# eriklindernoren/PyTorch-GAN

Measured on NVIDIA H100. Metric: DCGAN 64x64 images/sec (full G+D step), higher is better.
Workload: dtype tf32 (fp32 storage, fp32 accumulate)

## Files before the change

pytorch-gan_b200/csrc/narrow_block.cu:

```cuda
#include "tc_common.cuh"
#include <string.h>

namespace b200gan {

struct NbBn {
  const double *stats;
  const float *gamma, *beta;
  float eps;
  double count;
  int groups;
};

__device__ __forceinline__ void nb_bn_consts(const NbBn &bn, int C, int c, float &mean, float &rstd, float &sc,
                                             float &sh, double *var_out = nullptr, int grp = 0) {
  const double *st = bn.stats + (size_t)grp * 2 * C;
  const double m = st[c] / bn.count;
  double var = st[C + c] / bn.count - m * m;
  if (var < 0.0) var = 0.0;
  if (var_out) *var_out = var;
  rstd = (float)(1.0 / sqrt(var + (double)bn.eps));
  mean = (float)m;
  const float ga = bn.gamma ? bn.gamma[c] : 1.f, be = bn.beta ? bn.beta[c] : 0.f;
  sc = ga * rstd;
  sh = be - mean * sc;
// ... 6 lines not shown
    double var;
    nb_bn_consts(bn, C, c, mean, rstd, sc, sh, &var, grp);
    const double unbiased = bn.count > 1.0 ? var * bn.count / (bn.count - 1.0) : var;
    m_run = (1.f - momentum) * m_run + momentum * mean;
    v_run = (1.f - momentum) * v_run + momentum * (float)unbiased;
  }
  rm[c] = m_run;
  rv[c] = v_run;
}

__device__ __forceinline__ float nb_act(float v, int act, float slope) {
  if (act == B200GAN_ACT_LRELU) return v > 0.f ? v : v * slope;
  if (act == B200GAN_ACT_RELU) return fmaxf(v, 0.f);
  if (act == B200GAN_ACT_TANH) return tanhf(v);
  if (act == B200GAN_ACT_SIGMOID) return 1.f / (1.f + expf(-v));
  return v;
}
__device__ __forceinline__ float nb_act_grad(float a, int act, float slope) {
  if (act == B200GAN_ACT_LRELU) return a > 0.f ? 1.f : slope;
  if (act == B200GAN_ACT_RELU) return a > 0.f ? 1.f : 0.f;
  return 1.f;
}

__device__ __forceinline__ int ceil_div_dev(int a, int b) { return (a + b - 1) / b; }
__device__ __forceinline__ float warp_sum(float v) {
#pragma unroll
  for (int o = 16; o > 0; o >>= 1) v += __shfl_xor_sync(0xffffffffu, v, o);
  return v;
}

constexpr int NB_MAXC = 128;
constexpr int NB_MAX_GROUPS = 4;

__device__ __forceinline__ void nb_stage(float *dst, int CP, const float *src_img, int h0, int w0, int rows, int cols, int C,
                                         int H, int W, const float *sc_s, const float *sh_s, bool reflect, int tid) {
  if ((C & 3) == 0) {
    const int C4 = C >> 2, total = rows * cols * C4;
    for (int i = tid; i < total; i += 256) {
      const int c4 = i % C4, pix = i / C4;
      const int pc = pix % cols, pr = pix / cols;
      int ih = h0 + pr, iw = w0 + pc;
      if (reflect) {
        ih = reflect_idx(ih, H);
        iw = reflect_idx(iw, W);
      }
      float4 v = make_float4(0.f, 0.f, 0.f, 0.f);
      if (src_img && ih >= 0 && ih < H && iw >= 0 && iw < W) {
        v = __ldg(reinterpret_cast<const float4 *>(src_img + ((int64_t)ih * W + iw) * C) + c4);
        if (sc_s) {
          const float4 a = *reinterpret_cast<const float4 *>(sc_s + 4 * c4), b = *reinterpret_cast<const float4 *>(sh_s + 4 * c4);
          v.x = fmaf(v.x, a.x, b.x); v.y = fmaf(v.y, a.y, b.y); v.z = fmaf(v.z, a.z, b.z); v.w = fmaf(v.w, a.w, b.w);
        }
      }
      *reinterpret_cast<float4 *>(dst + (int64_t)pix * CP + 4 * c4) = v;
    }
  } else {
    const int total = rows * cols * C;
    for (int i = tid; i < total; i += 256) {
      const int cc = i % C, pix = i / C;
      const int pc = pix % cols, pr = pix / cols;
      int ih = h0 + pr, iw = w0 + pc;
      if (reflect) {
        ih = reflect_idx(ih, H);
        iw = reflect_idx(iw, W);
      }
      float v = 0.f;
      if (src_img && ih >= 0 && ih < H && iw >= 0 && iw < W) {
        v = __ldg(src_img + ((int64_t)ih * W + iw) * C + cc);
        if (sc_s) v = fmaf(v, sc_s[cc], sh_s[cc]);
      }
      dst[(int64_t)pix * CP + cc] = v;
    }
  }
}

struct NbTile {
  int TN, TR, TQ, TP, KG, KB;
  int tiles_r, tiles_q;
};

struct NbFprop2 {
  const float *x, *wp, *bias, *cs;
  float *y;
  double *out_stats;
  NbBn in_bn;
  float *rm, *rv;
  long long *nbt;
  float momentum;
  int N, H, W, C, P, Q, K, R, S, stride, pad_t, pad_l;
  float slope;
  int act;
  NbTile t;
  int PR, PC, CP;
  int reflect;
  int rtf;
  int groups;
};
template <int KT, int PT>
__global__ void __launch_bounds__(256)
nbk_fprop2_kernel(const __grid_constant__ NbFprop2 p) {
  extern __shared__ __align__(16) float nsm[];
  const NbTile &t = p.t;
  const int taps = p.R * p.S;
  float *w_s = nsm;
  float *x_s = w_s + (size_t)taps * p.C * t.KB;
  float *sc_s = x_s + (((size_t)t.TN * p.PR * p.PC * p.CP + 3) & ~(size_t)3);
  float *sh_s = sc_s + ((p.C + 3) & ~3);
  float *red = sh_s + ((p.C + 3) & ~3);
  const int tid = threadIdx.x, lane = tid & 31, warp = tid >> 5;
  const bool has_in = p.in_bn.stats != nullptr;
  const int grp = (int)((blockIdx.x / (t.tiles_q * t.tiles_r)) * t.TN) / (p.N / p.groups);
  for (int cc = tid; cc < p.C; cc += 256) {
    float mean, rstd, sc = 1.f, sh = 0.f;
    if (has_in) {
      nb_bn_consts(p.in_bn, p.C, cc, mean, rstd, sc, sh, nullptr, grp);
      if (blockIdx.x == 0 && blockIdx.y == 0 && p.rm) nb_update_running(p.in_bn, p.C, cc, p.rm, p.rv, p.momentum);
    }
    sc_s[cc] = sc;
    sh_s[cc] = sh;
  }
  if (has_in && blockIdx.x == 0 && blockIdx.y == 0 && tid == 0 && p.nbt) *p.nbt += p.in_bn.groups;
  const int kbase = blockIdx.y * t.KB;
  {
    const int KB4 = t.KB >> 2, total = taps * p.C * KB4;
#pragma unroll 4
    for (int i = tid; i < total; i += 256) {
      const int col = i % KB4, row = i / KB4;
      reinterpret_cast<float4 *>(w_s)[i] = __ldg(reinterpret_cast<const float4 *>(p.wp + (int64_t)row * p.K + kbase) + col);
    }
  }
  __syncthreads();
  int tile = blockIdx.x;
  const int tq = tile % t.tiles_q;
  tile /= t.tiles_q;
  const int tr = tile % t.tiles_r;
  const int n0 = (tile / t.tiles_r) * t.TN;
  const int p0 = tr * t.TR, q0 = tq * t.TQ;
  for (int li = 0; li < t.TN; ++li) {
    const int n = n0 + li;
    nb_stage(x_s + (size_t)li * p.PR * p.PC * p.CP, p.CP, n < p.N ? p.x + (int64_t)n * p.H * p.W * p.C : nullptr,
             p0 * p.stride - p.pad_t, q0 * p.stride - p.pad_l, p.PR, p.PC, p.C, p.H, p.W, has_in ? sc_s : nullptr, sh_s,
             p.reflect != 0, tid);
  }
  __syncthreads();

  const int TPX = t.TP / PT;
  const int lpx = tid % TPX, kgi = tid / TPX;
  int xoff[PT];
  int64_t yoff[PT];
  int nn[PT];
#pragma unroll
  for (int i = 0; i < PT; ++i) {
    const int lp = lpx + i * TPX;
    const int lq = lp % t.TQ, lr = (lp / t.TQ) % t.TR, li = lp / (t.TQ * t.TR);
    const int n = n0 + li, po = p0 + lr, qo = q0 + lq;
    xoff[i] = ((li * p.PR + lr * p.stride) * p.PC + lq * p.stride) * p.CP;
    nn[i] = n;
    yoff[i] = (n < p.N && po < p.P && qo < p.Q) ? ((int64_t)(n * p.P + po) * p.Q + qo) * p.K : -1;
  }
  float acc[PT][KT];
#pragma unroll
  for (int i = 0; i < PT; ++i)
#pragma unroll
    for (int j = 0; j < KT; ++j) acc[i][j] = 0.f;
  const float *wb = w_s + kgi * KT;
  const int KB = t.KB;
  for (int r = 0; r < p.R; ++r) {
    for (int s = 0; s < p.S; ++s) {
      const float *xt = x_s + (r * p.PC + s) * p.CP;
      const float *wt = wb + (size_t)(r * p.S + s) * p.C * KB;
      if ((p.C & 3) == 0) {
#pragma unroll 2
        for (int c = 0; c < p.C; c += 4) {
          float xs[PT][4];
#pragma unroll
          for (int i = 0; i < PT; ++i) {
            const float4 xv = *reinterpret_cast<const float4 *>(xt + xoff[i] + c);
// ... 6 lines not shown
            for (int u = 0; u < KT / 4; ++u) {
              const float4 w4 = *reinterpret_cast<const float4 *>(wr + 4 * u);
#pragma unroll
              for (int i = 0; i < PT; ++i) {
                acc[i][4 * u + 0] = fmaf(xs[i][j], w4.x, acc[i][4 * u + 0]);
                acc[i][4 * u + 1] = fmaf(xs[i][j], w4.y, acc[i][4 * u + 1]);
                acc[i][4 * u + 2] = fmaf(xs[i][j], w4.z, acc[i][4 * u + 2]);
                acc[i][4 * u + 3] = fmaf(xs[i][j], w4.w, acc[i][4 * u + 3]);
              }
            }
          }
        }
      } else {
        for (int c = 0; c < p.C; ++c) {
          float xs[PT];
#pragma unroll
          for (int i = 0; i < PT; ++i) xs[i] = xt[xoff[i] + c];
          const float *wr = wt + (size_t)c * KB;
#pragma unroll
          for (int u = 0; u < KT / 4; ++u) {
            const float4 w4 = *reinterpret_cast<const float4 *>(wr + 4 * u);
#pragma unroll
            for (int i = 0; i < PT; ++i) {
              acc[i][4 * u + 0] = fmaf(xs[i], w4.x, acc[i][4 * u + 0]);
              acc[i][4 * u + 1] = fmaf(xs[i], w4.y, acc[i][4 * u + 1]);
              acc[i][4 * u + 2] = fmaf(xs[i], w4.z, acc[i][4 * u + 2]);
              acc[i][4 * u + 3] = fmaf(xs[i], w4.w, acc[i][4 * u + 3]);
            }
          }
        }
      }
    }
  }
  const int k0 = kbase + kgi * KT;
  float s1[KT], s2[KT];
#pragma unroll
  for (int j = 0; j < KT; ++j) s1[j] = s2[j] = 0.f;
#pragma unroll
  for (int i = 0; i < PT; ++i) {
    const bool valid = yoff[i] >= 0;
#pragma unroll
    for (int j = 0; j < KT; ++j) {
      float v = acc[i][j];
      if (p.bias) v += __ldg(p.bias + k0 + j);
      v = nb_act(v, p.act, p.slope);
      if (p.cs && valid) v *= __ldg(p.cs + (int64_t)nn[i] * p.K + k0 + j);
      if (p.rtf) v = round_tf32(v);
      v = valid ? v : 0.f;
      acc[i][j] = v;
      s1[j] += v;
      s2[j] = fmaf(v, v, s2[j]);
    }
    if (valid) {
      float *yo = p.y + yoff[i] + k0;
#pragma unroll
      for (int u = 0; u < KT / 4; ++u)
        *reinterpret_cast<float4 *>(yo + 4 * u) =
            make_float4(acc[i][4 * u], acc[i][4 * u + 1], acc[i][4 * u + 2], acc[i][4 * u + 3]);
    }
  }
  if (p.out_stats) {
#pragma unroll
    for (int j = 0; j < KT; ++j) {
      const float a1 = warp_sum(s1[j]), a2 = warp_sum(s2[j]);
      if (lane == 0) {
        red[warp * 2 * KT + j] = a1;
        red[warp * 2 * KT + KT + j] = a2;
      }
    }
    __syncthreads();
    if (tid < t.KG * 2 * KT) {
      const int g = tid / (2 * KT), idx = tid % (2 * KT), wpg = TPX >> 5;
      float tsum = 0.f;
      for (int wi = 0; wi < wpg; ++wi) tsum += red[(g * wpg + wi) * 2 * KT + idx];
      atomicAdd(p.out_stats + (size_t)grp * 2 * p.K + (idx < KT ? 0 : p.K) + kbase + g * KT + (idx % KT), (double)tsum);
    }
  }
}

struct NbDz {
  const float *g, *a, *cs;
  float *dz, *db;
  NbBn out_bn;
  const double *sums;
  int64_t rows;
  int64_t PQ;
  int K;
  float slope;
  int act;
};
__global__ void __launch_bounds__(256)
nbk_dz_kernel(const __grid_constant__ NbDz p) {
  __shared__ float red[256][4];
  const int tid = threadIdx.x;
  const int K4 = p.K >> 2;
  const int kq = tid % K4;
  const int rows_per_block = 256 / K4;
  const bool has_bn = p.out_bn.stats != nullptr;
  const int grp = blockIdx.y;
  const int64_t grows = p.rows / gridDim.y, grow0 = grp * grows;
  float mean[4], rstd[4], sc[4], m1[4], m2[4];
#pragma unroll
  for (int j = 0; j < 4; ++j) {
    mean[j] = 0.f; rstd[j] = 0.f; sc[j] = 1.f; m1[j] = 0.f; m2[j] = 0.f;
    if (has_bn) {
      float sh;
      nb_bn_consts(p.out_bn, p.K, kq * 4 + j, mean[j], rstd[j], sc[j], sh, nullptr, grp);
      m1[j] = (float)(p.sums[(size_t)grp * 2 * p.K + kq * 4 + j] / p.out_bn.count);
      m2[j] = (float)(p.sums[(size_t)grp * 2 * p.K + p.K + kq * 4 + j] / p.out_bn.count);
    }
// ... 19 lines not shown
      o[j] = dA * csv[j] * nb_act_grad(A[j], p.act, p.slope);
      dbs[j] += o[j];
    }
    *reinterpret_cast<float4 *>(p.dz + off) = make_float4(o[0], o[1], o[2], o[3]);
  }
  if (p.db) {
#pragma unroll
    for (int j = 0; j < 4; ++j) red[tid][j] = dbs[j];
    __syncthreads();
    if (tid < K4) {
      float t4[4] = {0.f, 0.f, 0.f, 0.f};
      for (int r = 0; r < rows_per_block; ++r)
#pragma unroll
        for (int j = 0; j < 4; ++j) t4[j] += red[r * K4 + tid][j];
#pragma unroll
      for (int j = 0; j < 4; ++j) atomicAdd(p.db + tid * 4 + j, t4[j]);
    }
  }
}

struct NbWgrad {
  const float *x, *dz;
  float *dw;
  float *ws;
  int dw_elems;
  NbBn in_bn;
  int N, H, W, C, P, Q, K, R, S, stride, pad_t, pad_l;
  int TN, TR, TQ, tiles_r, tiles_q;
  int PR, PC;
  int SPB, PS;
  int nsets;
  int row_mode;
  int reflect;
};
template <int TAPS>
__global__ void __launch_bounds__(256, 2)
nbk_wgrad_kernel(const __grid_constant__ NbWgrad p) {
  extern __shared__ __align__(16) float nsm[];
  const int tile_px = p.TN * p.TR * p.TQ;
  const int K4 = (p.K + 3) >> 2, KP = K4 * 4;
  const int patch_img = p.PR * p.PC * p.C;
  int *sbase_s = reinterpret_cast<int *>(nsm);
  int *sk_s = sbase_s + p.SPB;
  int *poff_s = sk_s + p.SPB;
  float *x_s = nsm + ((2 * p.SPB + tile_px + 3) & ~3);
  float *dz_s = x_s + (((size_t)p.TN * patch_img + 3) & ~(size_t)3);
  const int Cr = (p.C + 3) & ~3;
  const int groups = p.in_bn.groups, img_per_group = p.N / groups;
  float *sc_s = dz_s + (size_t)tile_px * KP;
  float *sh_s = sc_s + (size_t)groups * Cr;
  const int tid = threadIdx.x;
  const bool has_in = p.in_bn.stats != nullptr;
  for (int i = tid; i < groups * p.C; i += 256) {
    const int gq = i / p.C, cc = i - gq * p.C;
    float mean, rstd, sc = 1.f, sh = 0.f;
    if (has_in) nb_bn_consts(p.in_bn, p.C, cc, mean, rstd, sc, sh, nullptr, gq);
    sc_s[gq * Cr + cc] = sc;
    sh_s[gq * Cr + cc] = sh;
  }
  for (int pix = tid; pix < tile_px; pix += 256) {
    const int lq = pix % p.TQ, lr = (pix / p.TQ) % p.TR, li = pix / (p.TQ * p.TR);
    poff_s[pix] = li * patch_img + ((lr * p.stride) * p.PC + lq * p.stride) * p.C;
  }
  const int RS = p.R * p.S;
  for (int sl = tid; sl < p.SPB; sl += 256) {
    const int set_o = blockIdx.y * p.SPB + sl;
    int base = -1, k0 = 0;
    if (set_o < p.nsets) {
      const int co = set_o % p.C, kgo = (set_o / p.C) % K4;
      const int ro = p.row_mode ? set_o / (p.C * K4) : 0;
      k0 = kgo * 4;
      base = (k0 * p.C + co) * RS + ro * p.S;
    }
    sbase_s[sl] = base;
    sk_s[sl] = k0;
  }
  const int set_local = tid & (p.SPB - 1), psplit = tid / p.SPB;
  const int set = blockIdx.y * p.SPB + set_local;
  const bool set_ok = set < p.nsets;
  const int c = set_ok ? set % p.C : 0, kg = set_ok ? (set / p.C) % K4 : 0;
  const int r_own = (set_ok && p.row_mode) ? set / (p.C * K4) : 0;
  float acc[TAPS][4];
#pragma unroll
  for (int t = 0; t < TAPS; ++t)
#pragma unroll
    for (int j = 0; j < 4; ++j) acc[t][j] = 0.f;
  const int ntiles = ceil_div_dev(p.N, p.TN) * p.tiles_r * p.tiles_q;
  int toff[TAPS];
#pragma unroll
  for (int t = 0; t < TAPS; ++t) toff[t] = p.row_mode ? (r_own * p.PC + t) * p.C : ((t / p.S) * p.PC + (t % p.S)) * p.C;
  __syncthreads();
  for (int tile = blockIdx.x; tile < ntiles; tile += gridDim.x) {
    const int tq = tile % p.tiles_q;
    const int tr = (tile / p.tiles_q) % p.tiles_r;
    const int n0 = (tile / (p.tiles_q * p.tiles_r)) * p.TN;
    const int p0 = tr * p.TR, q0 = tq * p.TQ;
    const int h0 = p0 * p.stride - p.pad_t, w0 = q0 * p.stride - p.pad_l;
    for (int li = 0; li < p.TN; ++li) {
      const int n = n0 + li;
      const int gq = n < p.N ? n / img_per_group : 0;
      nb_stage(x_s + (size_t)li * patch_img, p.C, n < p.N ? p.x + (int64_t)n * p.H * p.W * p.C : nullptr, h0, w0, p.PR, p.PC,
               p.C, p.H, p.W, has_in ? sc_s + gq * Cr : nullptr, sh_s + gq * Cr, p.reflect != 0, tid);
    }
    const int img_px = p.TR * p.TQ;
    if ((p.K & 3) == 0) {
      for (int i = tid; i < tile_px * K4; i += 256) {
        const int k4 = i % K4, pix = i / K4;
        const int li = pix / img_px, rem = pix - li * img_px;
        const int lr = rem / p.TQ, lq = rem - lr * p.TQ;
        float4 v = make_float4(0.f, 0.f, 0.f, 0.f);
        if (n0 + li < p.N && p0 + lr < p.P && q0 + lq < p.Q)
          v = __ldg(reinterpret_cast<const float4 *>(p.dz + ((int64_t)((n0 + li) * p.P + p0 + lr) * p.Q + q0 + lq) * p.K) + k4);
        reinterpret_cast<float4 *>(dz_s)[i] = v;
      }
    } else {
      for (int i = tid; i < tile_px * KP; i += 256) {
        const int k = i % KP, pix = i / KP;
        const int li = pix / img_px, rem = pix - li * img_px;
        const int lr = rem / p.TQ, lq = rem - lr * p.TQ;
        float v = 0.f;
        if (k < p.K && n0 + li < p.N && p0 + lr < p.P && q0 + lq < p.Q)
          v = __ldg(p.dz + ((int64_t)((n0 + li) * p.P + p0 + lr) * p.Q + q0 + lq) * p.K + k);
        dz_s[i] = v;
      }
    }
    __syncthreads();
    if (set_ok) {
      const float *xc = x_s + c;
      const float *dk = dz_s + kg * 4;
#pragma unroll 2
      for (int pix = psplit; pix < tile_px; pix += p.PS) {
        const float4 d4 = *reinterpret_cast<const float4 *>(dk + pix * KP);
        const float *xb = xc + poff_s[pix];
#pragma unroll
        for (int t = 0; t < TAPS; ++t) {
          const float xv = xb[toff[t]];
          acc[t][0] = fmaf(xv, d4.x, acc[t][0]);
          acc[t][1] = fmaf(xv, d4.y, acc[t][1]);
          acc[t][2] = fmaf(xv, d4.z, acc[t][2]);
          acc[t][3] = fmaf(xv, d4.w, acc[t][3]);
        }
      }
    }
    __syncthreads();
  }
  constexpr int TPAD = TAPS | 1;
  float *red = x_s;
#pragma unroll
  for (int j = 0; j < 4; ++j)
#pragma unroll
    for (int t = 0; t < TAPS; ++t) red[((size_t)(psplit * 4 + j) * p.SPB + set_local) * TPAD + t] = acc[t][j];
  __syncthreads();
  const int nout = 4 * p.SPB * TAPS;
  const int kstride = p.C * RS;
  float *slab = p.ws ? p.ws + (size_t)blockIdx.x * p.dw_elems : nullptr;
  for (int o = tid; o < nout; o += 256) {
    const int t = o % TAPS, rest = o / TAPS;
    const int sl = rest & (p.SPB - 1), j = rest / p.SPB;
    const int base = sbase_s[sl];
    if (base < 0) continue;
    if (sk_s[sl] + j >= p.K) continue;
    float sum = 0.f;
    for (int ps = 0; ps < p.PS; ++ps) sum += red[((size_t)(ps * 4 + j) * p.SPB + sl) * TPAD + t];
    const int idx = base + j * kstride + t;
    if (slab) slab[idx] = sum;
    else atomicAdd(p.dw + idx, sum);
  }
}

__global__ void __launch_bounds__(256)
nbk_wgrad_reduce_kernel(const float *__restrict__ ws, float *__restrict__ dw, int elems, int nslabs) {
  __shared__ float part[8][32];
  const int e = blockIdx.x * 32 + (threadIdx.x & 31), ph = threadIdx.x >> 5;
  float a = 0.f;
  if (e < elems) {
#pragma unroll 4
    for (int sl = ph; sl < nslabs; sl += 8) a += __ldg(ws + (size_t)sl * elems + e);
  }
  part[ph][threadIdx.x & 31] = a;
  __syncthreads();
  if (ph == 0 && e < elems) {
    float t = 0.f;
#pragma unroll
    for (int i = 0; i < 8; ++i) t += part[i][threadIdx.x];
    dw[e] = t;
  }
}

struct NbDgrad2 {
  const float *dz, *wp, *a_prev;
  float *g_out;
  double *sums;
  NbBn in_bn;
  int N, H, W, C, P, Q, K, R, S, stride, pad_t, pad_l;
  NbTile t;
  int KP;
  int PRm, PCm;
  int tapsm;
};
template <int KT, int PT>
__global__ void __launch_bounds__(256)
nbk_dgrad2_kernel(const __grid_constant__ NbDgrad2 p) {
  extern __shared__ __align__(16) float nsm[];
  const NbTile &t = p.t;
  float *w_s = nsm;
  float *d_s = w_s + (((size_t)p.tapsm * p.K * t.KB + 3) & ~(size_t)3);
  float *mean_s = d_s + (((size_t)t.TN * p.PRm * p.PCm * p.KP + 3) & ~(size_t)3);
  float *rstd_s = mean_s + ((p.C + 3) & ~3);
  float *red = rstd_s + ((p.C + 3) & ~3);
  const int tid = threadIdx.x, lane = tid & 31, warp = tid >> 5;
  const bool has_in = p.sums != nullptr;
  const int grp = (int)((blockIdx.x / (t.tiles_q * t.tiles_r)) * t.TN) / (p.N / p.in_bn.groups);
  if (has_in) {
    for (int cc = tid; cc < p.C; cc += 256) {
      float sc, sh;
      nb_bn_consts(p.in_bn, p.C, cc, mean_s[cc], rstd_s[cc], sc, sh, nullptr, grp);
    }
  }
  const int st = p.stride;
  const int cls = blockIdx.z;
  const int pa = cls / st, pb = cls % st;
  const int r0 = (pa + p.pad_t) % st, s0 = (pb + p.pad_l) % st;
  const int Rc = r0 < p.R ? (p.R - r0 + st - 1) / st : 0, Sc = s0 < p.S ? (p.S - s0 + st - 1) / st : 0;
  const int Hc = pa < p.H ? (p.H - pa + st - 1) / st : 0, Wc = pb < p.W ? (p.W - pb + st - 1) / st : 0;
  const int oh = (pa + p.pad_t - r0) / st, ow = (pb + p.pad_l - s0) / st;
  const int cbase = blockIdx.y * t.KB;
  const int KB = t.KB;
  if ((KB & 3) == 0) {
    const int KB4 = KB >> 2, total = Rc * Sc * p.K * KB4;
#pragma unroll 4
    for (int i = tid; i < total; i += 256) {
      const int col = i % KB4, row = i / KB4;
      const int k = row % p.K, ti = row / p.K;
      const int r = r0 + st * (ti / Sc), s_ = s0 + st * (ti % Sc);
      reinterpret_cast<float4 *>(w_s)[i] =
          __ldg(reinterpret_cast<const float4 *>(p.wp + ((int64_t)(r * p.S + s_) * p.K + k) * p.C + cbase) + col);
    }
  } else {
    const int total = Rc * Sc * p.K * KB;
    for (int i = tid; i < total; i += 256) {
      const int col = i % KB, row = i / KB;
      const int k = row % p.K, ti = row / p.K;
      const int r = r0 + st * (ti / Sc), s_ = s0 + st * (ti % Sc);
      w_s[i] = __ldg(p.wp + ((int64_t)(r * p.S + s_) * p.K + k) * p.C + cbase + col);
    }
  }
  int tile = blockIdx.x;
  const int tq = tile % t.tiles_q;
  tile /= t.tiles_q;
  const int tr = tile % t.tiles_r;
  const int n0 = (tile / t.tiles_r) * t.TN;
  const int i0 = tr * t.TR, j0 = tq * t.TQ;
  const int PRc = t.TR + (Rc > 0 ? Rc - 1 : 0), PCc = t.TQ + (Sc > 0 ? Sc - 1 : 0);
  for (int li = 0; li < t.TN; ++li) {
    const int n = n0 + li;
    nb_stage(d_s + (size_t)li * PRc * PCc * p.KP, p.KP, n < p.N ? p.dz + (int64_t)n * p.P * p.Q * p.K : nullptr,
             i0 + oh - (Rc - 1), j0 + ow - (Sc - 1), PRc, PCc, p.K, p.P, p.Q, nullptr, nullptr, false, tid);
  }
  __syncthreads();

  const int TPX = t.TP / PT;
  const int lpx = tid % TPX, cgi = tid / TPX;
  int doff[PT];
  int64_t opix[PT];
#pragma unroll
  for (int i = 0; i < PT; ++i) {
    const int lp = lpx + i * TPX;
    const int lq = lp % t.TQ, lr = (lp / t.TQ) % t.TR, li = lp / (t.TQ * t.TR);
    const int n = n0 + li, ci = i0 + lr, cj = j0 + lq;
    doff[i] = ((li * PRc + lr) * PCc + lq) * p.KP;
    opix[i] = (n < p.N && ci < Hc && cj < Wc) ? (int64_t)(n * p.H + pa + st * ci) * p.W + pb + st * cj : -1;
  }
  float acc[PT][KT];
#pragma unroll
  for (int i = 0; i < PT; ++i)
#pragma unroll
    for (int j = 0; j < KT; ++j) acc[i][j] = 0.f;
  const float *wb = w_s + cgi * KT;
  for (int ir = 0; ir < Rc; ++ir) {
    for (int is = 0; is < Sc; ++is) {
      const float *dt = d_s + ((Rc - 1 - ir) * PCc + (Sc - 1 - is)) * p.KP;
      const float *wt = wb + (size_t)(ir * Sc + is) * p.K * KB;
#pragma unroll 2
      for (int k = 0; k < p.K; k += 4) {
        float ds[PT][4];
#pragma unroll
        for (int i = 0; i < PT; ++i) {
          const float4 dv = *reinterpret_cast<const float4 *>(dt + doff[i] + k);
          ds[i][0] = dv.x; ds[i][1] = dv.y; ds[i][2] = dv.z; ds[i][3] = dv.w;
        }
#pragma unroll
        for (int j = 0; j < 4; ++j) {
          const float *wr = wt + (size_t)(k + j) * KB;
          if (KT % 4 == 0) {
#pragma unroll
            for (int u = 0; u < KT / 4; ++u) {
              const float4 w4 = *reinterpret_cast<const float4 *>(wr + 4 * u);
#pragma unroll
              for (int i = 0; i < PT; ++i) {
                acc[i][4 * u + 0] = fmaf(ds[i][j], w4.x, acc[i][4 * u + 0]);
                acc[i][4 * u + 1] = fmaf(ds[i][j], w4.y, acc[i][4 * u + 1]);
                acc[i][4 * u + 2] = fmaf(ds[i][j], w4.z, acc[i][4 * u + 2]);
                acc[i][4 * u + 3] = fmaf(ds[i][j], w4.w, acc[i][4 * u + 3]);
              }
            }
          } else {
#pragma unroll
            for (int u = 0; u < KT; ++u) {
              const float wv = wr[u];
#pragma unroll
              for (int i = 0; i < PT; ++i) acc[i][u] = fmaf(ds[i][j], wv, acc[i][u]);
            }
          }
        }
      }
    }
  }
  const int c0 = cbase + cgi * KT;
  float s1[KT], s2[KT];
#pragma unroll
  for (int j = 0; j < KT; ++j) s1[j] = s2[j] = 0.f;
#pragma unroll
  for (int i = 0; i < PT; ++i) {
    if (opix[i] < 0) continue;
    float *go = p.g_out + opix[i] * p.C + c0;
    if (KT % 4 == 0) {
#pragma unroll
      for (int u = 0; u < KT / 4; ++u)
        *reinterpret_cast<float4 *>(go + 4 * u) =
            make_float4(acc[i][4 * u], acc[i][4 * u + 1], acc[i][4 * u + 2], acc[i][4 * u + 3]);
    } else {
#pragma unroll
      for (int j = 0; j < KT; ++j) go[j] = acc[i][j];
    }
    if (has_in) {
      float ah[KT];
      if (KT % 4 == 0) {
#pragma unroll
        for (int u = 0; u < KT / 4; ++u) {
          const float4 a4 = __ldg(reinterpret_cast<const float4 *>(p.a_prev + opix[i] * p.C + c0) + u);
          ah[4 * u] = a4.x; ah[4 * u + 1] = a4.y; ah[4 * u + 2] = a4.z; ah[4 * u + 3] = a4.w;
        }
      } else {
#pragma unroll
        for (int j = 0; j < KT; ++j) ah[j] = __ldg(p.a_prev + opix[i] * p.C + c0 + j);
      }
#pragma unroll
      for (int j = 0; j < KT; ++j) {
        s1[j] += acc[i][j];
        s2[j] = fmaf(acc[i][j], (ah[j] - mean_s[c0 + j]) * rstd_s[c0 + j], s2[j]);
      }
    }
  }
  if (has_in) {
#pragma unroll
    for (int j = 0; j < KT; ++j) {
      const float a1 = warp_sum(s1[j]), a2 = warp_sum(s2[j]);
      if (lane == 0) {
        red[warp * 2 * KT + j] = a1;
        red[warp * 2 * KT + KT + j] = a2;
      }
    }
    __syncthreads();
    if (tid < t.KG * 2 * KT) {
      const int g = tid / (2 * KT), idx = tid % (2 * KT), wpg = TPX >> 5;
      float tsum = 0.f;
      for (int wi = 0; wi < wpg; ++wi) tsum += red[(g * wpg + wi) * 2 * KT + idx];
      atomicAdd(p.sums + (size_t)grp * 2 * p.C + (idx < KT ? 0 : p.C) + cbase + g * KT + (idx % KT), (double)tsum);
    }
  }
}

struct NbTail {
  const float *a;
  const float *dout;
  float *out;
  float *g;
  double *sums;
  NbBn bn;
  float *rm, *rv;
  long long *nbt;
  float momentum;
  int N, HW, C, nchw;
};
__global__ void __launch_bounds__(256)
nbk_tail_fwd_kernel(const __grid_constant__ NbTail p) {
  __shared__ float sc_s[NB_MAXC], sh_s[NB_MAXC];
  const int tid = threadIdx.x;
  const int grp = blockIdx.y;
  if (tid < p.C) {
    float mean, rstd;
    nb_bn_consts(p.bn, p.C, tid, mean, rstd, sc_s[tid], sh_s[tid], nullptr, grp);
    if (blockIdx.x == 0 && grp == 0 && p.rm) nb_update_running(p.bn, p.C, tid, p.rm, p.rv, p.momentum);
  }
  if (blockIdx.x == 0 && grp == 0 && tid == 0 && p.nbt) *p.nbt += p.bn.groups;
  __syncthreads();
  const int64_t gtotal = (int64_t)(p.N / gridDim.y) * p.HW * p.C, total = (grp + 1) * gtotal;
  for (int64_t i = grp * gtotal + (int64_t)blockIdx.x * 256 + tid; i < total; i += (int64_t)gridDim.x * 256) {
    int c;
    int64_t src;
    if (p.nchw) {
      const int hw = (int)(i % p.HW);
      c = (int)((i / p.HW) % p.C);
// ... 173 lines not shown
  X(3, 2) X(3, 4) X(1, 1)
#define NB_IS_INSTANCE(KT_, PT_) if (pl.KT == KT_ && pl.PT == PT_) return true;
static bool nb_fprop_instance(const NbPlan &pl) {
  NB_FPROP_INSTANCES(NB_IS_INSTANCE)
  return false;
}
static bool nb_dgrad_instance(const NbPlan &pl) {
  NB_DGRAD_INSTANCES(NB_IS_INSTANCE)
  return false;
}
#undef NB_IS_INSTANCE

static int nb_fprop2_launch(const b200gan_conv_geom *g, const NbBn &in_bn, float *rm, float *rv, long long *nbt,
                            float momentum, const float *x, const float *packed, const float *bias, int act, float slope,
                            const float *chan_scale, float *y, double *out_stats, int reflect, int rtf, int groups,
                            cudaStream_t st) {
  B2_CHECK_ARG(groups >= 1 && groups <= NB_MAX_GROUPS && g->N % groups == 0, "nb_fprop: bad statistics group count");
  const NbPlan pl = nb_plan_fprop(g, groups);
  B2_CHECK_ARG(pl.ok, "nb_fprop: no tile plan fits in shared memory");
  B2_CHECK_ARG(nb_fprop_instance(pl), "nb_fprop: no kernel instance for KT=%d PT=%d", pl.KT, pl.PT);
  if (out_stats) B2_CUDA(cudaMemsetAsync(out_stats, 0, (size_t)groups * 2 * g->K * sizeof(double), st));
  NbFprop2 q;
  q.x = x; q.wp = packed; q.bias = bias; q.cs = chan_scale; q.y = y; q.out_stats = out_stats;
  q.in_bn = in_bn; q.rm = rm; q.rv = rv; q.nbt = nbt; q.momentum = momentum;
  q.N = g->N; q.H = g->H; q.W = g->W; q.C = g->C; q.P = g->P; q.Q = g->Q; q.K = g->K; q.R = g->R; q.S = g->S;
  q.stride = g->stride; q.pad_t = g->pad_t; q.pad_l = g->pad_l; q.slope = slope; q.act = act;
  q.t = pl.t;
  q.PR = (pl.t.TR - 1) * g->stride + g->R;
  q.PC = (pl.t.TQ - 1) * g->stride + g->S;
  q.CP = (g->C % 4 == 0) ? g->C + 4 : g->C;
  q.reflect = reflect;
  q.rtf = rtf;
  q.groups = groups;
  dim3 grid((unsigned)(ceil_div(g->N, pl.t.TN) * pl.t.tiles_r * pl.t.tiles_q), (unsigned)(g->K / pl.t.KB));
#define NB_FPROP_CASE(KT_, PT_)                                                                              \
  if (pl.KT == KT_ && pl.PT == PT_) {                                                                        \
    static std::atomic<uint64_t> done{0};                                                                    \
    if (int e = ensure_dynamic_smem(nbk_fprop2_kernel<KT_, PT_>, (int)NB_SMEM_MAX, done)) return e;          \
    nbk_fprop2_kernel<KT_, PT_><<<grid, 256, pl.smem, st>>>(q);                                              \
  }
  NB_FPROP_INSTANCES(NB_FPROP_CASE)
#undef NB_FPROP_CASE
  B2_LAUNCH_CHECK();
  return B200GAN_OK;
}

bool nb_plain_fprop_ok(const b200gan_conv_geom *g) {
  if (!g || g->transposed || g->up != 1) return false;
  if (g->pad_mode != B200GAN_PAD_ZERO && g->pad_mode != B200GAN_PAD_REFLECT) return false;
  if (g->stride != 1 && g->stride != 2) return false;
  if (g->C < 1 || g->C > 8 || g->K < 16 || g->K > NB_MAXC || g->K % 16 != 0) return false;
  if (g->R != g->S || (g->R != 3 && g->R != 4 && g->R != 7)) return false;
  return nb_plan_fprop(g).ok;
}
int nb_plain_fprop(const b200gan_conv_geom *g, const b200gan_epilogue *ep, const float *x, const float *packed, float *y,
                   cudaStream_t st) {
  if ((int64_t)g->N * g->P * g->Q == 0) return B200GAN_OK;
  NbBn none = to_bn(nullptr);
  return nb_fprop2_launch(g, none, nullptr, nullptr, nullptr, 0.f, x, packed, ep ? ep->bias : nullptr,
                          ep ? ep->act : B200GAN_ACT_NONE, ep ? ep->slope : 0.f, ep ? ep->chan_scale : nullptr, y, nullptr,
                          g->pad_mode == B200GAN_PAD_REFLECT ? 1 : 0, ep ? ep->round_tf32 : 0, 1, st);
}
}

extern "C" int b200gan_nb_fprop(const b200gan_conv_geom *g, const b200gan_nb_bn *in_bn, float *running_mean,
                                float *running_var, int64_t *num_batches_tracked, float momentum, const float *x,
// ... 118 lines not shown
  B2_CHECK_ARG(validate_geom(g) == B200GAN_OK && nb_wgrad_ok(g), "nb_wgrad: unsupported geometry");
  B2_CHECK_ARG(x && dz && dw, "nb_wgrad: null pointer");
  return nb_wgrad_run(g, in_bn, x, dz, dw, workspace, as_stream(stream));
}

int b200gan::nb_wgrad_run(const b200gan_conv_geom *g, const b200gan_nb_bn *in_bn, const float *x, const float *dz,
                          float *dw, float *workspace, cudaStream_t st) {
  const int dw_elems = g->K * g->C * g->R * g->S;
  if ((int64_t)g->N * g->P * g->Q == 0) {
    B2_CUDA(cudaMemsetAsync(dw, 0, (size_t)dw_elems * sizeof(float), st));
    return B200GAN_OK;
  }
  const int groups = (in_bn && in_bn->stats && in_bn->groups > 1) ? in_bn->groups : 1;
  B2_CHECK_ARG(g->N % groups == 0, "nb_wgrad: the batch must split evenly into the statistics groups");
  B2_CHECK_ARG(groups == 1 || (groups <= NB_MAX_GROUPS && g->C <= NB_MAXC), "nb_wgrad: too many statistics groups");
  const NbWgPlan w = nb_wgrad_plan(g);
  B2_CHECK_ARG(w.smem <= 96 * 1024, "nb_wgrad: tile does not fit in shared memory");
  const bool use_ws = w.use_ws && workspace != nullptr;
  if (!use_ws) B2_CUDA(cudaMemsetAsync(dw, 0, (size_t)dw_elems * sizeof(float), st));
  NbWgrad p;
  p.x = x; p.dz = dz; p.dw = dw; p.ws = use_ws ? workspace : nullptr; p.dw_elems = dw_elems; p.in_bn = to_bn(in_bn);
  p.N = g->N; p.H = g->H; p.W = g->W; p.C = g->C; p.P = g->P; p.Q = g->Q; p.K = g->K; p.R = g->R; p.S = g->S;
  p.stride = g->stride; p.pad_t = g->pad_t; p.pad_l = g->pad_l;
  p.TN = w.TN; p.TR = w.TR; p.TQ = w.TQ;
  p.tiles_r = ceil_div(g->P, p.TR);
  p.tiles_q = ceil_div(g->Q, p.TQ);
  p.PR = (p.TR - 1) * g->stride + g->R;
  p.PC = (p.TQ - 1) * g->stride + g->S;
  p.row_mode = w.row_mode;
  p.reflect = g->pad_mode == B200GAN_PAD_REFLECT ? 1 : 0;
  p.nsets = w.nsets;
  p.SPB = w.SPB;
  p.PS = w.PS;
  const int taps = g->R * g->S;
  static std::atomic<uint64_t> done9{0}, done16{0}, done7{0};
  dim3 grid((unsigned)w.gx, (unsigned)w.nchunks);
  if (p.row_mode) {
    if (int e = ensure_dynamic_smem(nbk_wgrad_kernel<7>, 96 * 1024, done7)) return e;
    nbk_wgrad_kernel<7><<<grid, 256, w.smem, st>>>(p);
  } else if (taps == 9) {
    if (int e = ensure_dynamic_smem(nbk_wgrad_kernel<9>, 96 * 1024, done9)) return e;
    nbk_wgrad_kernel<9><<<grid, 256, w.smem, st>>>(p);
  } else {
    if (int e = ensure_dynamic_smem(nbk_wgrad_kernel<16>, 96 * 1024, done16)) return e;
    nbk_wgrad_kernel<16><<<grid, 256, w.smem, st>>>(p);
  }
  B2_LAUNCH_CHECK();
  if (use_ws) return nb_wgrad_reduce(workspace, dw, dw_elems, w.gx, st);
  return B200GAN_OK;
}

int b200gan::nb_wgrad_reduce(const float *ws, float *dw, int elems, int nslabs, cudaStream_t st) {
  nbk_wgrad_reduce_kernel<<<(unsigned)ceil_div(elems, 32), 256, 0, st>>>(ws, dw, elems, nslabs);
  B2_LAUNCH_CHECK();
  return B200GAN_OK;
}

namespace b200gan {
static int nb_dgrad2_launch(const b200gan_conv_geom *g, const float *dz, const float *packed, const NbBn &in_bn,
                            const float *a_prev, float *g_out, double *sums, cudaStream_t st) {
  const int st_ = g->stride;
  const int groups = in_bn.stats ? in_bn.groups : 1;
  B2_CHECK_ARG(groups <= NB_MAX_GROUPS && g->N % groups == 0, "nb_dgrad: bad statistics group count");
  const NbPlan pl = nb_plan_dgrad(g, groups);
  B2_CHECK_ARG(pl.ok, "nb_dgrad: no tile plan fits in shared memory");
  B2_CHECK_ARG(nb_dgrad_instance(pl), "nb_dgrad: no kernel instance for KT=%d PT=%d", pl.KT, pl.PT);
  if (sums) B2_CUDA(cudaMemsetAsync(sums, 0, (size_t)groups * 2 * g->C * sizeof(double), st));
  NbDgrad2 q;
  q.dz = dz; q.wp = packed; q.a_prev = a_prev; q.g_out = g_out; q.sums = sums; q.in_bn = in_bn;
  q.N = g->N; q.H = g->H; q.W = g->W; q.C = g->C; q.P = g->P; q.Q = g->Q; q.K = g->K; q.R = g->R; q.S = g->S;
  q.stride = g->stride; q.pad_t = g->pad_t; q.pad_l = g->pad_l;
  q.t = pl.t;
  q.KP = g->K + 4;
  const int Rm = ceil_div(g->R, st_), Sm = ceil_div(g->S, st_);
  q.PRm = pl.t.TR + Rm - 1;
  q.PCm = pl.t.TQ + Sm - 1;
  q.tapsm = Rm * Sm;
  dim3 grid((unsigned)(ceil_div(g->N, pl.t.TN) * pl.t.tiles_r * pl.t.tiles_q), (unsigned)(g->C / pl.t.KB),
            (unsigned)(st_ * st_));
#define NB_DGRAD_CASE(KT_, PT_)                                                                              \
  if (pl.KT == KT_ && pl.PT == PT_) {                                                                        \
    static std::atomic<uint64_t> done{0};                                                                    \
    if (int e = ensure_dynamic_smem(nbk_dgrad2_kernel<KT_, PT_>, (int)NB_SMEM_MAX, done)) return e;          \
    nbk_dgrad2_kernel<KT_, PT_><<<grid, 256, pl.smem, st>>>(q);                                              \
  }
  NB_DGRAD_INSTANCES(NB_DGRAD_CASE)
#undef NB_DGRAD_CASE
  B2_LAUNCH_CHECK();
  return B200GAN_OK;
}

bool nb_plain_dgrad_ok(const b200gan_conv_geom *g) {
  if (!g || g->transposed || g->up != 1 || g->pad_mode != B200GAN_PAD_ZERO) return false;
  if (g->stride != 1 && g->stride != 2) return false;
  if (g->pad_t != g->pad_b || g->pad_l != g->pad_r) return false;
  if (g->C < 1 || g->C > 8 || (g->C != 1 && g->C != 3 && g->C != 6 && g->C % 4 != 0)) return false;
  if (g->K < 4 || g->K > NB_MAXC || g->K % 4 != 0) return false;
  if (g->R * g->S != 9 && g->R * g->S != 16 && !(g->R == 7 && g->S == 7 && g->stride == 1)) return false;
  return nb_plan_dgrad(g).ok;
}
int nb_plain_dgrad(const b200gan_conv_geom *g, const float *dy, const float *packed, float *dx, cudaStream_t st) {
  if ((int64_t)g->N * g->H * g->W == 0) return B200GAN_OK;
  NbBn none = to_bn(nullptr);
  return nb_dgrad2_launch(g, dy, packed, none, nullptr, dx, nullptr, st);
}
}

extern "C" int b200gan_nb_dgrad(const b200gan_conv_geom *g, const float *dz, const float *packed,
                                const b200gan_nb_bn *in_bn, const float *a_prev, float *g_out, double *sums,
                                void *stream) {
// ... 55 lines not shown
```

Baseline: 47140.

## Stage conv tiles with cp.async and overlap loads with BN constant setup

Replaces register-staged global→shared copies of weights, input patches and dz in the narrow-block fprop, wgrad and dgrad kernels with cp.async transfers, issuing them before the per-channel BN constant computation so the two overlap. Input normalization is split into a second in-shared-memory pass after the copy completes, which costs an extra shared read/write and sync when BN is applied. It also adds compile-time-gated clock tracing hooks and an incremental index helper to avoid per-element divisions.

```diff
diff --git a/pytorch-gan_b200/csrc/narrow_block.cu b/pytorch-gan_b200/csrc/narrow_block.cu
--- a/pytorch-gan_b200/csrc/narrow_block.cu
+++ b/pytorch-gan_b200/csrc/narrow_block.cu
@@ -62,44 +62,93 @@
 constexpr int NB_MAXC = 128;
 constexpr int NB_MAX_GROUPS = 4;
 
-__device__ __forceinline__ void nb_stage(float *dst, int CP, const float *src_img, int h0, int w0, int rows, int cols, int C,
-                                         int H, int W, const float *sc_s, const float *sh_s, bool reflect, int tid) {
-  if ((C & 3) == 0) {
-    const int C4 = C >> 2, total = rows * cols * C4;
-    for (int i = tid; i < total; i += 256) {
-      const int c4 = i % C4, pix = i / C4;
-      const int pc = pix % cols, pr = pix / cols;
-      int ih = h0 + pr, iw = w0 + pc;
-      if (reflect) {
-        ih = reflect_idx(ih, H);
-        iw = reflect_idx(iw, W);
-      }
-      float4 v = make_float4(0.f, 0.f, 0.f, 0.f);
-      if (src_img && ih >= 0 && ih < H && iw >= 0 && iw < W) {
-        v = __ldg(reinterpret_cast<const float4 *>(src_img + ((int64_t)ih * W + iw) * C) + c4);
-        if (sc_s) {
-          const float4 a = *reinterpret_cast<const float4 *>(sc_s + 4 * c4), b = *reinterpret_cast<const float4 *>(sh_s + 4 * c4);
-          v.x = fmaf(v.x, a.x, b.x); v.y = fmaf(v.y, a.y, b.y); v.z = fmaf(v.z, a.z, b.z); v.w = fmaf(v.w, a.w, b.w);
-        }
-      }
-      *reinterpret_cast<float4 *>(dst + (int64_t)pix * CP + 4 * c4) = v;
-    }
-  } else {
-    const int total = rows * cols * C;
-    for (int i = tid; i < total; i += 256) {
-      const int cc = i % C, pix = i / C;
-      const int pc = pix % cols, pr = pix / cols;
-      int ih = h0 + pr, iw = w0 + pc;
-      if (reflect) {
-        ih = reflect_idx(ih, H);
-        iw = reflect_idx(iw, W);
-      }
-      float v = 0.f;
-      if (src_img && ih >= 0 && ih < H && iw >= 0 && iw < W) {
-        v = __ldg(src_img + ((int64_t)ih * W + iw) * C + cc);
-        if (sc_s) v = fmaf(v, sc_s[cc], sh_s[cc]);
-      }
-      dst[(int64_t)pix * CP + cc] = v;
+#ifdef NB_TRACE
+constexpr int NB_TRACE_SLOTS = 8;
+static long long *g_nb_trace = nullptr;
+extern "C" void b200gan_nb_set_trace(void *buf) { g_nb_trace = reinterpret_cast<long long *>(buf); }
+__device__ __forceinline__ long long *nb_trace_slot(long long *tr) {
+  return tr + (((size_t)blockIdx.z * gridDim.y + blockIdx.y) * gridDim.x + blockIdx.x) * NB_TRACE_SLOTS;
+}
+__device__ __forceinline__ long long nb_clock_sync() {
+  __syncthreads();
+  return clock64();
+}
+#define NB_TRACE_FIELD long long *trace;
+#define NB_TRACE_SET(q) (q).trace = g_nb_trace
+#define NB_MARK(slot)                                                                  \
+  do {                                                                                 \
+    const long long clk_ = nb_clock_sync();                                            \
+    if (p.trace && threadIdx.x == 0) nb_trace_slot(p.trace)[slot] = clk_;              \
+  } while (0)
+#else
+#define NB_TRACE_FIELD
+#define NB_TRACE_SET(q) (void)0
+#define NB_MARK(slot) (void)0
+#endif
+
+__device__ __forceinline__ void cp_async16(float *dst, const float *src, int src_bytes) {
+  asm volatile("cp.async.cg.shared.global [%0], [%1], 16, %2;" ::"r"((unsigned)__cvta_generic_to_shared(dst)), "l"(src),
+               "r"(src_bytes)
+               : "memory");
+}
+__device__ __forceinline__ void cp_async4(float *dst, const float *src, int src_bytes) {
+  asm volatile("cp.async.ca.shared.global [%0], [%1], 4, %2;" ::"r"((unsigned)__cvta_generic_to_shared(dst)), "l"(src),
+               "r"(src_bytes)
+               : "memory");
+}
+__device__ __forceinline__ void cp_async_wait_all() { asm volatile("cp.async.wait_all;" ::: "memory"); }
+
+struct NbIdx {
+  int col, row, dc, dr;
+  __device__ __forceinline__ NbIdx(int n, int tid) : col(tid % n), row(tid / n), dc(256 % n), dr(256 / n) {}
+  __device__ __forceinline__ void next(int n) {
+    col += dc;
+    row += dr;
+    if (col >= n) {
+      col -= n;
+      ++row;
+    }
+  }
+};
+
+__device__ __forceinline__ void nb_stage_issue(float *dst, int CP, const float *src_img, int h0, int w0, int rows, int cols,
+                                               int C, int H, int W, bool reflect, int tid) {
+  const bool vec = (C & 3) == 0;
+  const int CV = vec ? C >> 2 : C, npix = rows * cols;
+  for (NbIdx ix(CV, tid); ix.row < npix; ix.next(CV)) {
+    const int pr = ix.row / cols, pc = ix.row - pr * cols;
+    int ih = h0 + pr, iw = w0 + pc;
+    if (reflect) {
+      ih = reflect_idx(ih, H);
+      iw = reflect_idx(iw, W);
+    }
+    const bool in = src_img && ih >= 0 && ih < H && iw >= 0 && iw < W;
+    float *d = dst + (int64_t)ix.row * CP;
+    if (vec) {
+      const float *s = in ? src_img + ((int64_t)ih * W + iw) * C + 4 * ix.col : dst;
+      cp_async16(d + 4 * ix.col, s, in ? 16 : 0);
+    } else {
+      const float *s = in ? src_img + ((int64_t)ih * W + iw) * C + ix.col : dst;
+      cp_async4(d + ix.col, s, in ? 4 : 0);
+    }
+  }
+}
+__device__ __forceinline__ void nb_stage_norm(float *dst, int CP, int h0, int w0, int rows, int cols, int C, int H, int W,
+                                              const float *sc_s, const float *sh_s, bool reflect, int tid) {
+  const bool vec = (C & 3) == 0;
+  const int CV = vec ? C >> 2 : C, npix = rows * cols;
+  for (NbIdx ix(CV, tid); ix.row < npix; ix.next(CV)) {
+    const int pr = ix.row / cols, pc = ix.row - pr * cols;
+    const int ih = h0 + pr, iw = w0 + pc;
+    if (!reflect && (ih < 0 || ih >= H || iw < 0 || iw >= W)) continue;
+    float *d = dst + (int64_t)ix.row * CP;
+    if (vec) {
+      float4 v = *reinterpret_cast<float4 *>(d + 4 * ix.col);
+      const float4 a = *reinterpret_cast<const float4 *>(sc_s + 4 * ix.col), b = *reinterpret_cast<const float4 *>(sh_s + 4 * ix.col);
+      v.x = fmaf(v.x, a.x, b.x); v.y = fmaf(v.y, a.y, b.y); v.z = fmaf(v.z, a.z, b.z); v.w = fmaf(v.w, a.w, b.w);
+      *reinterpret_cast<float4 *>(d + 4 * ix.col) = v;
+    } else {
+      d[ix.col] = fmaf(d[ix.col], sc_s[ix.col], sh_s[ix.col]);
     }
   }
 }
@@ -125,6 +174,7 @@
   int reflect;
   int rtf;
   int groups;
+  NB_TRACE_FIELD
 };
 template <int KT, int PT>
 __global__ void __launch_bounds__(256)
@@ -139,6 +189,27 @@
   float *red = sh_s + ((p.C + 3) & ~3);
   const int tid = threadIdx.x, lane = tid & 31, warp = tid >> 5;
   const bool has_in = p.in_bn.stats != nullptr;
+  NB_MARK(0);
+  NB_MARK(1);
+  int tile = blockIdx.x;
+  const int tq = tile % t.tiles_q;
+  tile /= t.tiles_q;
+  const int tr = tile % t.tiles_r;
+  const int n0 = (tile / t.tiles_r) * t.TN;
+  const int p0 = tr * t.TR, q0 = tq * t.TQ;
+  const int h0 = p0 * p.stride - p.pad_t, w0 = q0 * p.stride - p.pad_l;
+  const size_t win = (size_t)p.PR * p.PC * p.CP;
+  const int kbase = blockIdx.y * t.KB;
+  {
+    const int KB4 = t.KB >> 2;
+    for (NbIdx ix(KB4, tid); ix.row < taps * p.C; ix.next(KB4))
+      cp_async16(w_s + ((size_t)ix.row * KB4 + ix.col) * 4, p.wp + (int64_t)ix.row * p.K + kbase + 4 * ix.col, 16);
+  }
+  for (int li = 0; li < t.TN; ++li) {
+    const int n = n0 + li;
+    nb_stage_issue(x_s + li * win, p.CP, n < p.N ? p.x + (int64_t)n * p.H * p.W * p.C : nullptr, h0, w0, p.PR, p.PC,
+                   p.C, p.H, p.W, p.reflect != 0, tid);
+  }
   const int grp = (int)((blockIdx.x / (t.tiles_q * t.tiles_r)) * t.TN) / (p.N / p.groups);
   for (int cc = tid; cc < p.C; cc += 256) {
     float mean, rstd, sc = 1.f, sh = 0.f;
@@ -150,29 +221,15 @@
     sh_s[cc] = sh;
   }
   if (has_in && blockIdx.x == 0 && blockIdx.y == 0 && tid == 0 && p.nbt) *p.nbt += p.in_bn.groups;
-  const int kbase = blockIdx.y * t.KB;
-  {
-    const int KB4 = t.KB >> 2, total = taps * p.C * KB4;
-#pragma unroll 4
-    for (int i = tid; i < total; i += 256) {
-      const int col = i % KB4, row = i / KB4;
-      reinterpret_cast<float4 *>(w_s)[i] = __ldg(reinterpret_cast<const float4 *>(p.wp + (int64_t)row * p.K + kbase) + col);
-    }
-  }
+  NB_MARK(2);
+  cp_async_wait_all();
   __syncthreads();
-  int tile = blockIdx.x;
-  const int tq = tile % t.tiles_q;
-  tile /= t.tiles_q;
-  const int tr = tile % t.tiles_r;
-  const int n0 = (tile / t.tiles_r) * t.TN;
-  const int p0 = tr * t.TR, q0 = tq * t.TQ;
-  for (int li = 0; li < t.TN; ++li) {
-    const int n = n0 + li;
-    nb_stage(x_s + (size_t)li * p.PR * p.PC * p.CP, p.CP, n < p.N ? p.x + (int64_t)n * p.H * p.W * p.C : nullptr,
-             p0 * p.stride - p.pad_t, q0 * p.stride - p.pad_l, p.PR, p.PC, p.C, p.H, p.W, has_in ? sc_s : nullptr, sh_s,
-             p.reflect != 0, tid);
-  }
-  __syncthreads();
+  if (has_in) {
+    for (int li = 0; li < t.TN && n0 + li < p.N; ++li)
+      nb_stage_norm(x_s + li * win, p.CP, h0, w0, p.PR, p.PC, p.C, p.H, p.W, sc_s, sh_s, p.reflect != 0, tid);
+    __syncthreads();
+  }
+  NB_MARK(3);
 
   const int TPX = t.TP / PT;
   const int lpx = tid % TPX, kgi = tid / TPX;
@@ -245,6 +302,7 @@
       }
     }
   }
+  NB_MARK(4);
   const int k0 = kbase + kgi * KT;
   float s1[KT], s2[KT];
 #pragma unroll
@@ -289,6 +347,7 @@
       atomicAdd(p.out_stats + (size_t)grp * 2 * p.K + (idx < KT ? 0 : p.K) + kbase + g * KT + (idx % KT), (double)tsum);
     }
   }
+  NB_MARK(5);
 }
 
 struct NbDz {
@@ -374,6 +433,7 @@
   int nsets;
   int row_mode;
   int reflect;
+  NB_TRACE_FIELD
 };
 template <int TAPS>
 __global__ void __launch_bounds__(256, 2)
@@ -393,6 +453,7 @@
   float *sh_s = sc_s + (size_t)groups * Cr;
   const int tid = threadIdx.x;
   const bool has_in = p.in_bn.stats != nullptr;
+  NB_MARK(0);
   for (int i = tid; i < groups * p.C; i += 256) {
     const int gq = i / p.C, cc = i - gq * p.C;
     float mean, rstd, sc = 1.f, sh = 0.f;
@@ -432,6 +493,10 @@
 #pragma unroll
   for (int t = 0; t < TAPS; ++t) toff[t] = p.row_mode ? (r_own * p.PC + t) * p.C : ((t / p.S) * p.PC + (t % p.S)) * p.C;
   __syncthreads();
+  NB_MARK(1);
+#ifdef NB_TRACE
+  long long tr_stage = 0, tr_fma = 0, tr_tiles = 0, tr_t = clock64();
+#endif
   for (int tile = blockIdx.x; tile < ntiles; tile += gridDim.x) {
     const int tq = tile % p.tiles_q;
     const int tr = (tile / p.tiles_q) % p.tiles_r;
@@ -440,33 +505,35 @@
     const int h0 = p0 * p.stride - p.pad_t, w0 = q0 * p.stride - p.pad_l;
     for (int li = 0; li < p.TN; ++li) {
       const int n = n0 + li;
-      const int gq = n < p.N ? n / img_per_group : 0;
-      nb_stage(x_s + (size_t)li * patch_img, p.C, n < p.N ? p.x + (int64_t)n * p.H * p.W * p.C : nullptr, h0, w0, p.PR, p.PC,
-               p.C, p.H, p.W, has_in ? sc_s + gq * Cr : nullptr, sh_s + gq * Cr, p.reflect != 0, tid);
+      nb_stage_issue(x_s + (size_t)li * patch_img, p.C, n < p.N ? p.x + (int64_t)n * p.H * p.W * p.C : nullptr, h0, w0,
+                     p.PR, p.PC, p.C, p.H, p.W, p.reflect != 0, tid);
     }
     const int img_px = p.TR * p.TQ;
-    if ((p.K & 3) == 0) {
-      for (int i = tid; i < tile_px * K4; i += 256) {
-        const int k4 = i % K4, pix = i / K4;
-        const int li = pix / img_px, rem = pix - li * img_px;
+    {
+      const bool vec = (p.K & 3) == 0;
+      const int KV = vec ? K4 : KP;
+      for (NbIdx ix(KV, tid); ix.row < tile_px; ix.next(KV)) {
+        const int pix = ix.row, li = pix / img_px, rem = pix - li * img_px;
         const int lr = rem / p.TQ, lq = rem - lr * p.TQ;
-        float4 v = make_float4(0.f, 0.f, 0.f, 0.f);
-        if (n0 + li < p.N && p0 + lr < p.P && q0 + lq < p.Q)
-          v = __ldg(reinterpret_cast<const float4 *>(p.dz + ((int64_t)((n0 + li) * p.P + p0 + lr) * p.Q + q0 + lq) * p.K) + k4);
-        reinterpret_cast<float4 *>(dz_s)[i] = v;
+        const bool in = n0 + li < p.N && p0 + lr < p.P && q0 + lq < p.Q && (vec || ix.col < p.K);
+        const float *src = in ? p.dz + ((int64_t)((n0 + li) * p.P + p0 + lr) * p.Q + q0 + lq) * p.K : p.dz;
+        if (vec) cp_async16(dz_s + ((size_t)pix * K4 + ix.col) * 4, src + (in ? 4 * ix.col : 0), in ? 16 : 0);
+        else cp_async4(dz_s + (size_t)pix * KP + ix.col, src + (in ? ix.col : 0), in ? 4 : 0);
       }
-    } else {
-      for (int i = tid; i < tile_px * KP; i += 256) {
-        const int k = i % KP, pix = i / KP;
-        const int li = pix / img_px, rem = pix - li * img_px;
-        const int lr = rem / p.TQ, lq = rem - lr * p.TQ;
-        float v = 0.f;
-        if (k < p.K && n0 + li < p.N && p0 + lr < p.P && q0 + lq < p.Q)
-          v = __ldg(p.dz + ((int64_t)((n0 + li) * p.P + p0 + lr) * p.Q + q0 + lq) * p.K + k);
-        dz_s[i] = v;
+    }
+    cp_async_wait_all();
+    __syncthreads();
+    if (has_in) {
+      for (int li = 0; li < p.TN && n0 + li < p.N; ++li) {
+        const int gq = (n0 + li) / img_per_group;
+        nb_stage_norm(x_s + (size_t)li * patch_img, p.C, h0, w0, p.PR, p.PC, p.C, p.H, p.W, sc_s + gq * Cr, sh_s + gq * Cr,
+                      p.reflect != 0, tid);
       }
-    }
-    __syncthreads();
+      __syncthreads();
+    }
+#ifdef NB_TRACE
+    { const long long c_ = nb_clock_sync(); tr_stage += c_ - tr_t; tr_t = c_; ++tr_tiles; }
+#endif
     if (set_ok) {
       const float *xc = x_s + c;
       const float *dk = dz_s + kg * 4;
@@ -485,7 +552,16 @@
       }
     }
     __syncthreads();
-  }
+#ifdef NB_TRACE
+    { const long long c_ = nb_clock_sync(); tr_fma += c_ - tr_t; tr_t = c_; }
+#endif
+  }
+#ifdef NB_TRACE
+  if (p.trace && tid == 0) {
+    long long *tr_ = nb_trace_slot(p.trace);
+    tr_[2] = tr_stage; tr_[3] = tr_fma; tr_[6] = tr_tiles;
+  }
+#endif
   constexpr int TPAD = TAPS | 1;
   float *red = x_s;
 #pragma unroll
@@ -508,6 +584,7 @@
     if (slab) slab[idx] = sum;
     else atomicAdd(p.dw + idx, sum);
   }
+  NB_MARK(5);
 }
 
 __global__ void __launch_bounds__(256)
@@ -539,6 +616,7 @@
   int KP;
   int PRm, PCm;
   int tapsm;
+  NB_TRACE_FIELD
 };
 template <int KT, int PT>
 __global__ void __launch_bounds__(256)
@@ -552,13 +630,8 @@
   float *red = rstd_s + ((p.C + 3) & ~3);
   const int tid = threadIdx.x, lane = tid & 31, warp = tid >> 5;
   const bool has_in = p.sums != nullptr;
-  const int grp = (int)((blockIdx.x / (t.tiles_q * t.tiles_r)) * t.TN) / (p.N / p.in_bn.groups);
-  if (has_in) {
-    for (int cc = tid; cc < p.C; cc += 256) {
-      float sc, sh;
-      nb_bn_consts(p.in_bn, p.C, cc, mean_s[cc], rstd_s[cc], sc, sh, nullptr, grp);
-    }
-  }
+  NB_MARK(0);
+  NB_MARK(1);
   const int st = p.stride;
   const int cls = blockIdx.z;
   const int pa = cls / st, pb = cls % st;
@@ -568,23 +641,16 @@
   const int oh = (pa + p.pad_t - r0) / st, ow = (pb + p.pad_l - s0) / st;
   const int cbase = blockIdx.y * t.KB;
   const int KB = t.KB;
-  if ((KB & 3) == 0) {
-    const int KB4 = KB >> 2, total = Rc * Sc * p.K * KB4;
-#pragma unroll 4
-    for (int i = tid; i < total; i += 256) {
-      const int col = i % KB4, row = i / KB4;
-      const int k = row % p.K, ti = row / p.K;
-      const int r = r0 + st * (ti / Sc), s_ = s0 + st * (ti % Sc);
-      reinterpret_cast<float4 *>(w_s)[i] =
-          __ldg(reinterpret_cast<const float4 *>(p.wp + ((int64_t)(r * p.S + s_) * p.K + k) * p.C + cbase) + col);
-    }
-  } else {
-    const int total = Rc * Sc * p.K * KB;
-    for (int i = tid; i < total; i += 256) {
-      const int col = i % KB, row = i / KB;
-      const int k = row % p.K, ti = row / p.K;
-      const int r = r0 + st * (ti / Sc), s_ = s0 + st * (ti % Sc);
-      w_s[i] = __ldg(p.wp + ((int64_t)(r * p.S + s_) * p.K + k) * p.C + cbase + col);
+  {
+    const bool vec = (KB & 3) == 0;
+    const int KBV = vec ? KB >> 2 : KB;
+    for (NbIdx ix(KBV, tid); ix.row < Rc * Sc * p.K; ix.next(KBV)) {
+      const int ti = ix.row / p.K, k = ix.row - ti * p.K;
+      const int tr_ = ti / Sc;
+      const int r = r0 + st * tr_, s_ = s0 + st * (ti - tr_ * Sc);
+      const float *src = p.wp + ((int64_t)(r * p.S + s_) * p.K + k) * p.C + cbase;
+      if (vec) cp_async16(w_s + ((size_t)ix.row * KBV + ix.col) * 4, src + 4 * ix.col, 16);
+      else cp_async4(w_s + (size_t)ix.row * KB + ix.col, src + ix.col, 4);
     }
   }
   int tile = blockIdx.x;
@@ -596,10 +662,20 @@
   const int PRc = t.TR + (Rc > 0 ? Rc - 1 : 0), PCc = t.TQ + (Sc > 0 ? Sc - 1 : 0);
   for (int li = 0; li < t.TN; ++li) {
     const int n = n0 + li;
-    nb_stage(d_s + (size_t)li * PRc * PCc * p.KP, p.KP, n < p.N ? p.dz + (int64_t)n * p.P * p.Q * p.K : nullptr,
-             i0 + oh - (Rc - 1), j0 + ow - (Sc - 1), PRc, PCc, p.K, p.P, p.Q, nullptr, nullptr, false, tid);
-  }
+    nb_stage_issue(d_s + (size_t)li * PRc * PCc * p.KP, p.KP, n < p.N ? p.dz + (int64_t)n * p.P * p.Q * p.K : nullptr,
+                   i0 + oh - (Rc - 1), j0 + ow - (Sc - 1), PRc, PCc, p.K, p.P, p.Q, false, tid);
+  }
+  const int grp = (int)((blockIdx.x / (t.tiles_q * t.tiles_r)) * t.TN) / (p.N / p.in_bn.groups);
+  if (has_in) {
+    for (int cc = tid; cc < p.C; cc += 256) {
+      float sc, sh;
+      nb_bn_consts(p.in_bn, p.C, cc, mean_s[cc], rstd_s[cc], sc, sh, nullptr, grp);
+    }
+  }
+  NB_MARK(2);
+  cp_async_wait_all();
   __syncthreads();
+  NB_MARK(3);
 
   const int TPX = t.TP / PT;
   const int lpx = tid % TPX, cgi = tid / TPX;
@@ -658,6 +734,7 @@
       }
     }
   }
+  NB_MARK(4);
   const int c0 = cbase + cgi * KT;
   float s1[KT], s2[KT];
 #pragma unroll
@@ -711,6 +788,7 @@
       atomicAdd(p.sums + (size_t)grp * 2 * p.C + (idx < KT ? 0 : p.C) + cbase + g * KT + (idx % KT), (double)tsum);
     }
   }
+  NB_MARK(5);
 }
 
 struct NbTail {
@@ -950,6 +1028,7 @@
   q.reflect = reflect;
   q.rtf = rtf;
   q.groups = groups;
+  NB_TRACE_SET(q);
   dim3 grid((unsigned)(ceil_div(g->N, pl.t.TN) * pl.t.tiles_r * pl.t.tiles_q), (unsigned)(g->K / pl.t.KB));
 #define NB_FPROP_CASE(KT_, PT_)                                                                              \
   if (pl.KT == KT_ && pl.PT == PT_) {                                                                        \
@@ -1134,6 +1213,7 @@
   p.nsets = w.nsets;
   p.SPB = w.SPB;
   p.PS = w.PS;
+  NB_TRACE_SET(p);
   const int taps = g->R * g->S;
   static std::atomic<uint64_t> done9{0}, done16{0}, done7{0};
   dim3 grid((unsigned)w.gx, (unsigned)w.nchunks);
@@ -1178,6 +1258,7 @@
   q.PRm = pl.t.TR + Rm - 1;
   q.PCm = pl.t.TQ + Sm - 1;
   q.tapsm = Rm * Sm;
+  NB_TRACE_SET(q);
   dim3 grid((unsigned)(ceil_div(g->N, pl.t.TN) * pl.t.tiles_r * pl.t.tiles_q), (unsigned)(g->C / pl.t.KB),
             (unsigned)(st_ * st_));
 #define NB_DGRAD_CASE(KT_, PT_)                                                                              \
```

Result: faster. 47940 (median of 6 runs) (+1.7%).
